# wielgosz-info/pedestrians-video-2-carla

Measured on AMD Instinct MI355X. Metric: clips/sec (B=256,T=16,J=26) pose_lifting train step, higher is better.
Workload: dtype f32; 1 GPU; flow=pose_lifting movements_model=LinearAE(pose_changes) loss=loc_2d_3d transform=hips_neck_bbox clip_length=16 J=26 batch_size=256/GPU (BASELINE.json metric config; configs[1]/[3] = --batch-size 1024); global_batch=256, per_gpu_batch=256, parallelism=dp1, hip_graph=True, lean_train_outputs=True, deferred_loss_finalize=True, two_launch_step=True, direct_replay=True, grad_allreduce_bytes=70120

## Files before the change

pedestrians_video_2_carla_amd/csrc/p2c_pose_head_dev.h:

```cpp
#pragma once
#include <hip/hip_runtime.h>
#include <stdint.h>
#include <math.h>

#include "../../include/p2c.h"

namespace p2c {

constexpr int J = P2C_JOINTS;
constexpr int GROUP = 32;
constexpr int IDL = 26;

static __constant__ int c_parent[GROUP] = {IDL, 0, 1, 2, 3, 4, 5, 6, 3, 8, 9, 9, 3, 12, 13, 14, 1, 16, 17, 18, 19, 1, 21, 22, 23, 24,
                                    26, 27, 28, 29, 30, 31};
static __constant__ int c_subtree_end[GROUP] = {25, 25, 15, 15, 7, 7, 7, 7, 11, 11, 10, 11, 15, 15, 15, 15, 20, 20, 20, 20, 20,
                                         25, 25, 25, 25, 25, 26, 27, 28, 29, 30, 31};
constexpr unsigned kInteriorMask = 0x3dee6feu;
static __constant__ int c_anc_r2[GROUP] = {26, 26, 0, 1, 2, 3, 4, 5, 3, 3, 8, 9, 3, 3, 12, 13, 1, 1, 16, 17, 18, 1, 1, 21, 22, 23,
                                    26, 27, 28, 29, 30, 31};
static __constant__ int c_anc_r3[GROUP] = {26, 26, 26, 26, 0, 1, 2, 3, 1, 1, 3, 3, 1, 1, 3, 3, 26, 26, 1, 1, 16, 26, 26, 1, 1, 21,
                                    26, 27, 28, 29, 30, 31};

struct V3 {
  float x, y, z;
// ... 61 lines not shown
#pragma unroll
  for (int i = 0; i < 9; ++i) c.m[i] = shfl(a.m[i], s);
  return c;
}
template <int CTRL, int ROW_MASK = 0xF>
__device__ __forceinline__ float dpp0(float v) {
  return __int_as_float(__builtin_amdgcn_update_dpp(0, __float_as_int(v), CTRL, ROW_MASK, 0xF, true));
}
__device__ __forceinline__ float group_prefix(float v) {
  v += dpp0<0x111>(v);
  v += dpp0<0x112>(v);
  v += dpp0<0x114>(v);
  v += dpp0<0x118>(v);
  v += dpp0<0x142, 0xA>(v);
  return v;
}
__device__ __forceinline__ float group_bcast(float v, int j, bool upper) {
  float lo = __int_as_float(__builtin_amdgcn_readlane(__float_as_int(v), j));
  float hi = __int_as_float(__builtin_amdgcn_readlane(__float_as_int(v), j + 32));
  return upper ? hi : lo;
}
__device__ __forceinline__ float group_sum(float v, bool upper) { return group_bcast(group_prefix(v), 31, upper); }
__device__ __forceinline__ float group_min(float v) {
#pragma unroll
  for (int d = 16; d >= 1; d >>= 1) v = fminf(v, __shfl_xor(v, d, 64));
  return v;
}
__device__ __forceinline__ float group_max(float v) {
#pragma unroll
  for (int d = 16; d >= 1; d >>= 1) v = fmaxf(v, __shfl_xor(v, d, 64));
  return v;
}
__device__ __forceinline__ float wave_sum(float v) {
#pragma unroll
  for (int d = 32; d >= 1; d >>= 1) v += __shfl_xor(v, d, 64);
  return v;
}

__device__ __forceinline__ float frcp(float x) { return __builtin_amdgcn_rcpf(x); }
__device__ __forceinline__ float fsqrt(float x) { return __builtin_amdgcn_sqrtf(x); }

__device__ __forceinline__ float nan_to_zero(float v) { return (isfinite(v)) ? v : 0.f; }

struct SixD {
  V3 a1, a2, b1, b2;
  float n1, n2, d;
  bool c1, c2;
};
__device__ __forceinline__ M3 rot6d_fwd(const float *y6, SixD &s) {
  s.a1 = v3(y6[0], y6[1], y6[2]);
  s.a2 = v3(y6[3], y6[4], y6[5]);
  float n1 = fsqrt(dot(s.a1, s.a1));
  s.c1 = n1 > 1e-12f;
  s.n1 = fmaxf(n1, 1e-12f);
  s.b1 = s.a1 * frcp(s.n1);
  s.d = dot(s.b1, s.a2);
  V3 u2 = s.a2 - s.b1 * s.d;
  float n2 = fsqrt(dot(u2, u2));
  s.c2 = n2 > 1e-12f;
  s.n2 = fmaxf(n2, 1e-12f);
  s.b2 = u2 * frcp(s.n2);
  V3 b3 = cross(s.b1, s.b2);
  return M3{{s.b1.x, s.b1.y, s.b1.z, s.b2.x, s.b2.y, s.b2.z, b3.x, b3.y, b3.z}};
}
__device__ __forceinline__ void rot6d_bwd(const SixD &s, const M3 &g, float *gy6) {
  V3 g1 = v3(g.m[0], g.m[1], g.m[2]), g2 = v3(g.m[3], g.m[4], g.m[5]), g3 = v3(g.m[6], g.m[7], g.m[8]);
  V3 gb1 = g1 + cross(s.b2, g3);
  V3 gb2 = g2 + cross(g3, s.b1);
// ... 64 lines not shown
    V3 l1 = vmul(l, Ra) + la;
    M3 R1 = mul(R, Ra);
    if (L.interior) {
      l = l1;
      R = R1;
    }
  }
  {
    M3 Ra = shfl(R, L.base + L.anc1);
    V3 la = shfl(l, L.base + L.anc1);
    l = vmul(l, Ra) + la;
    R = mul(R, Ra);
  }
  {
    M3 Ra = shfl(R, L.base + L.anc2);
    V3 la = shfl(l, L.base + L.anc2);
    l = vmul(l, Ra) + la;
    if (NEED_ROT) R = mul(R, Ra);
  }
}

struct World {
  M3 rot;
  V3 loc;
  bool on;
};

struct HeadAcc {
  float sum2, cnt2, sum3;
};

enum { MODE_FWD = 0, MODE_FWD_MATERIALIZE = 1, MODE_BWD = 2, MODE_TRAIN = 3 };

template <int MODE>
__device__ __forceinline__ V3 frame_head(const p2c_pose_head_desc &d, const LaneCtx &L, int t, V3 x, const World &W,
                                         HeadAcc &acc, float coef2, float coef3, const float *g_abs_ext,
                                         const float *g_projt_ext, const float *gt2v, const float *gt3v) {
  constexpr bool BWD = (MODE == MODE_BWD || MODE == MODE_TRAIN);
  constexpr bool SUMS = !BWD || MODE == MODE_TRAIN;
  constexpr bool MAT = (MODE == MODE_FWD_MATERIALIZE);
  const bool in_slice = (t >= d.t0) && (t < d.t1);
  const size_t frame = (size_t)L.clip * d.T + t;

  V3 w = v3(x.y, -x.x, x.z);
  V3 p = W.on ? vmul(w, W.rot) + W.loc : w;
  float Z = d.cam_dist - p.x;
  float invZ = frcp(Z);
  float u = d.cam_cx - d.cam_f * p.y * invZ;
  float v = d.cam_cy + d.cam_f * (p.z + d.cam_elev) * invZ;
  if (!L.active) { u = 0.f; v = 0.f; invZ = 0.f; }

  if (MAT) {
    if (L.active && d.out_projection_2d) {
      float *o = d.out_projection_2d + (frame * J + L.j) * 3;
      o[0] = u, o[1] = v, o[2] = invZ;
    }
    if (L.active && d.out_absolute_pose_loc) {
      float *o = d.out_absolute_pose_loc + (frame * J + L.j) * 3;
      o[0] = x.x, o[1] = x.y, o[2] = x.z;
    }
  }

  const int tr = d.transform;
  float su = 0.f, sv = 0.f, scale = 1.f;
  float hu = 0.f, hv = 0.f, ku = 0.f, kv = 0.f;
  float hn_scale = 1.f, bb_scale = 1.f;
  bool use_bb_scale = false;
  float minu = 0.f, maxu = 0.f, minv = 0.f, maxv = 0.f;
  bool missing = false;
  if (tr != P2C_TRANSFORM_NONE) {
    if (tr != P2C_TRANSFORM_BBOX) {
      const bool up = L.base != 0;
      hu = group_bcast(u, d.hips_idx[0], up);
      hv = group_bcast(v, d.hips_idx[0], up);
      if (d.n_hips == 2) {
        hu = 0.5f * (hu + group_bcast(u, d.hips_idx[1], up));
        hv = 0.5f * (hv + group_bcast(v, d.hips_idx[1], up));
      }
      ku = group_bcast(u, d.neck_idx[0], up);
      kv = group_bcast(v, d.neck_idx[0], up);
      if (d.n_neck == 2) {
        ku = 0.5f * (ku + group_bcast(u, d.neck_idx[1], up));
        kv = 0.5f * (kv + group_bcast(v, d.neck_idx[1], up));
      }
      float du = ku - hu, dv = kv - hv;
// ... 9 lines not shown
    }
    if (__any(need_bb)) {
      missing = !L.active || ((u < d.near_zero) && (v < d.near_zero)) || (L.j >= J);
      const float inf = __builtin_inff();
      minu = group_min(missing ? inf : u);
      minv = group_min(missing ? inf : v);
      maxu = group_max(missing ? -inf : u);
      maxv = group_max(missing ? -inf : v);
      float cu = 0.5f * (minu + maxu), cv = 0.5f * (minv + maxv);
      float top_v = fminf(minv, maxv);
      float dx = cu - cu, dy = top_v - cv;
      bb_scale = fsqrt(fmaf(dx, dx, dy * dy));
      if (tr == P2C_TRANSFORM_BBOX) {
        su = cu, sv = cv, scale = bb_scale;
      } else if (use_bb_scale) {
        scale = bb_scale * 0.5748f;
      }
    }
  }
  float nu = u, nv = v, wch = invZ;
  bool fin_u = true, fin_v = true, keep = true;
  float inv_scale = 1.f;
  if (tr != P2C_TRANSFORM_NONE) {
    inv_scale = frcp(scale);
    nu = (u - su) * inv_scale;
    nv = (v - sv) * inv_scale;
    fin_u = isfinite(nu), fin_v = isfinite(nv);
    nu = fin_u ? nu : 0.f;
    nv = fin_v ? nv : 0.f;
    wch = nan_to_zero(invZ);
    keep = wch >= d.near_zero;
    if (!keep) { nu = 0.f; nv = 0.f; }
  }
  if (MAT && tr != P2C_TRANSFORM_NONE && in_slice && L.clip < d.B) {
    if (L.active && d.out_projection_2d_transformed) {
      float *o = d.out_projection_2d_transformed + (frame * J + L.j) * 3;
      o[0] = nu, o[1] = nv, o[2] = wch;
    }
    if (L.j == 0) {
      if (d.out_shift) d.out_shift[frame * 2 + 0] = su, d.out_shift[frame * 2 + 1] = sv;
      if (d.out_scale) d.out_scale[frame] = scale;
    }
  }

  V3 gx = v3(0.f, 0.f, 0.f);
  float dnu = 0.f, dnv = 0.f;
  if (in_slice) {
    if (L.has2) {
      float g0 = gt2v[0], g1 = gt2v[1];
      bool m = !d.mask_missing_joints || L.never_masked || ((g0 != 0.f) && (g1 != 0.f));
      if (m) {
        float e0 = nu - g0, e1 = nv - g1;
        if (SUMS) {
          acc.sum2 += fmaf(e0, e0, e1 * e1);
          acc.cnt2 += 1.f;
        }
        if (BWD) {
          dnu = coef2 * e0;
          dnv = coef2 * e1;
        }
      }
    }
    if (L.has3) {
      float e0 = x.x - gt3v[0], e1 = x.y - gt3v[1], e2 = x.z - gt3v[2];
      if (SUMS) acc.sum3 += fmaf(e0, e0, fmaf(e1, e1, e2 * e2));
      if (BWD) gx = v3(coef3 * e0, coef3 * e1, coef3 * e2);
    }
  }
  if (!BWD) return gx;

  if (L.active && g_abs_ext) {
    const float *g = g_abs_ext + (frame * J + L.j) * 3;
    gx = gx + v3(g[0], g[1], g[2]);
  }
// ... 33 lines not shown
    if (tr == P2C_TRANSFORM_BBOX || __any(use_bb_scale)) {
      float g_minu = 0.f, g_maxu = 0.f, g_minv = 0.f, g_maxv = 0.f;
      if (tr == P2C_TRANSFORM_BBOX) {
        g_minu += 0.5f * gsu, g_maxu += 0.5f * gsu, g_minv += 0.5f * gsv, g_maxv += 0.5f * gsv;
      }
      if (tr == P2C_TRANSFORM_BBOX || use_bb_scale) {
        float dy = fminf(minv, maxv) - 0.5f * (minv + maxv);
        float g_dy = (bb_scale > 0.f) ? g_bbs * dy * frcp(bb_scale) : 0.f;
        g_minv += 0.5f * g_dy;
        g_maxv -= 0.5f * g_dy;
      }
      unsigned long long grp = 0xffffffffull << L.base;
      unsigned long long b;
      b = __ballot(!missing && u == minu) & grp;
      if (b && L.lane == __ffsll((long long)b) - 1) gu += g_minu;
      b = __ballot(!missing && u == maxu) & grp;
      if (b && L.lane == __ffsll((long long)b) - 1) gu += g_maxu;
      b = __ballot(!missing && v == minv) & grp;
      if (b && L.lane == __ffsll((long long)b) - 1) gv += g_minv;
      b = __ballot(!missing && v == maxv) & grp;
      if (b && L.lane == __ffsll((long long)b) - 1) gv += g_maxv;
    }
  }
  float fz = d.cam_f * invZ;
  float gb = -fz * gu;
  float gc = fz * gv;
  float gZ = (d.cam_f * p.y * gu - d.cam_f * (p.z + d.cam_elev) * gv) * invZ * invZ;
  V3 gp = v3(-gZ, gb, gc);
  V3 gw = W.on ? vmulT(gp, W.rot) : gp;
  if (L.active) gx = gx + v3(-gw.y, gw.x, gw.z);
  return gx;
}

__device__ __forceinline__ void world_step(const p2c_pose_head_desc &d, const LaneCtx &L, int t, World &W) {
  if (!W.on || L.clip >= d.B) return;
  size_t frame = (size_t)L.clip * d.T + t;
  if (d.drot) {
    M3 dr;
#pragma unroll
    for (int i = 0; i < 9; ++i) dr.m[i] = d.drot[frame * 9 + i];
    W.rot = d.world_absolute ? dr : mul(W.rot, dr);
  }
  if (d.dloc) {
    V3 dl = v3(d.dloc[frame * 3 + 0], d.dloc[frame * 3 + 1], d.dloc[frame * 3 + 2]);
    W.loc = d.world_absolute ? dl : W.loc + dl;
  }
}
__device__ __forceinline__ void world_store(const p2c_pose_head_desc &d, const LaneCtx &L, int t, const World &W) {
  if (L.j != 0 || L.clip >= d.B) return;
  size_t frame = (size_t)L.clip * d.T + t;
  if (d.out_world_loc) {
    d.out_world_loc[frame * 3 + 0] = W.loc.x, d.out_world_loc[frame * 3 + 1] = W.loc.y, d.out_world_loc[frame * 3 + 2] = W.loc.z;
  }
  if (d.out_world_rot) {
#pragma unroll
    for (int i = 0; i < 9; ++i) d.out_world_rot[frame * 9 + i] = W.rot.m[i];
  }
}

struct GradLosses {
  const float *p[3];
};
__device__ __forceinline__ void loss_coefs_n(const p2c_pose_head_desc &d, const GradLosses &gl, float n2, float n3,
                                             float &coef2, float &coef3) {
  if (!gl.p[0] && !gl.p[1] && !gl.p[2]) return;
  const float u0 = gl.p[0] ? *gl.p[0] : 0.f, u1 = gl.p[1] ? *gl.p[1] : 0.f, u2 = gl.p[2] ? *gl.p[2] : 0.f;
  float g2 = u0 + u2, g3 = u1 + u2;
// ... 112 lines not shown
typedef float fb_f32x4 __attribute__((ext_vector_type(4)));
template <int NY, int DIR>
__device__ __forceinline__ void load_frame(const LaneCtx &L, FramePtrs &p, FrameIn<NY> &f) {
  (void)L;
  if constexpr (NY == 6) {
    const fb_f32x4 a = __builtin_bit_cast(fb_f32x4, __builtin_amdgcn_raw_buffer_load_b128(p.y, p.oy, 0, 0));
    const fb_f32x2 b = __builtin_bit_cast(fb_f32x2, __builtin_amdgcn_raw_buffer_load_b64(p.y, p.oy + 16, 0, 0));
    f.y[0] = a[0], f.y[1] = a[1], f.y[2] = a[2], f.y[3] = a[3], f.y[4] = b[0], f.y[5] = b[1];
  } else if constexpr (NY == 9) {
    const fb_f32x4 a = __builtin_bit_cast(fb_f32x4, __builtin_amdgcn_raw_buffer_load_b128(p.y, p.oy, 0, 0));
    const fb_f32x4 b = __builtin_bit_cast(fb_f32x4, __builtin_amdgcn_raw_buffer_load_b128(p.y, p.oy + 16, 0, 0));
    const float c = __builtin_bit_cast(float, __builtin_amdgcn_raw_buffer_load_b32(p.y, p.oy + 32, 0, 0));
    f.y[0] = a[0], f.y[1] = a[1], f.y[2] = a[2], f.y[3] = a[3];
    f.y[4] = b[0], f.y[5] = b[1], f.y[6] = b[2], f.y[7] = b[3], f.y[8] = c;
  } else {
    static_assert(NY == 3, "frame inputs are 6-D rotations, 3x3 matrices or 3-D locations");
    const fb_f32x3 a = __builtin_bit_cast(fb_f32x3, __builtin_amdgcn_raw_buffer_load_b96(p.y, p.oy, 0, 0));
    f.y[0] = a[0], f.y[1] = a[1], f.y[2] = a[2];
  }
  const fb_f32x2 g2 = __builtin_bit_cast(fb_f32x2, __builtin_amdgcn_raw_buffer_load_b64(p.g2, p.o2, 0, 0));
  const fb_f32x3 g3 = __builtin_bit_cast(fb_f32x3, __builtin_amdgcn_raw_buffer_load_b96(p.g3, p.o3, 0, 0));
  f.g2[0] = g2[0], f.g2[1] = g2[1];
  f.g3[0] = g3[0], f.g3[1] = g3[1], f.g3[2] = g3[2];
  p.oy += DIR * p.sy, p.o2 += DIR * p.s2, p.o3 += DIR * p.s3;
}

__device__ __forceinline__ void store_m3(float *base, size_t idx, const M3 &a) {
  float *p = base + idx * 9;
#pragma unroll
  for (int i = 0; i < 9; ++i) p[i] = a.m[i];
}


__device__ __forceinline__ World world_at(const p2c_pose_head_desc &d, const LaneCtx &L, int t) {
  World W;
  W.on = (d.dloc != nullptr) || (d.drot != nullptr);
  W.rot = identity();
  W.loc = v3(0.f, 0.f, 0.f);
  if (W.on) {
    const int tt = t < d.T ? t : d.T - 1;
    if (d.world_absolute) world_step(d, L, tt, W);
    else
      for (int i = 0; i <= tt; ++i) world_step(d, L, i, W);
  }
  return W;
}

__device__ __forceinline__ M3 scan_time(M3 P, int t, int j, int T, float *planes, int plane_floats) {
  int cur = 0;
  for (int off = 1; off < T; off <<= 1) {
    float *mine = planes + cur * plane_floats + (t * GROUP + j) * 9;
#pragma unroll
    for (int i = 0; i < 9; ++i) mine[i] = P.m[i];
    __syncthreads();
    if (t >= off) {
      const float *q = planes + cur * plane_floats + ((t - off) * GROUP + j) * 9;
      M3 Q;
#pragma unroll
      for (int i = 0; i < 9; ++i) Q.m[i] = q[i];
      P = mul(P, Q);
    }
    cur ^= 1;
  }
  return P;
}

__device__ __forceinline__ float n3_elems(const p2c_pose_head_desc &d) {
// ... 42 lines not shown
```

pedestrians_video_2_carla_amd/csrc/p2c_train.hip:

```cpp
#include <hip/hip_runtime.h>
#include <stdlib.h>
#include <stdint.h>

#include "../../include/p2c.h"
#include "p2c_adam_math.h"
#include "p2c_mlp_dev.h"
#include "p2c_pose_head_dev.h"
#include "p2c_train_dev.h"

int p2c_internal_validate_pose_head(const p2c_pose_head_desc *d);

namespace p2c_train {

constexpr int T_MAX = TS;
constexpr int PLANE = T_MAX * ph::GROUP * 9;
constexpr int H_ROWS = S::h_off(NLAY);
constexpr int G_ROWS = S::act_rows() - S::h_off(1);
constexpr int ACT_FLOATS = (H_ROWS + G_ROWS) * TP;
static_assert((S::h_off(NLAY) - S::h_off(1)) * TP >= PLANE, "scan plane 1 aliases the rows of G_1 .. G_{L-1}");
static_assert(S::dim_at(NLAY) == ph::J * 6, "the last layer is the (26, 6) rotation output");
constexpr int SCRATCH = 64;
constexpr int LDS_FLOATS = S::w_total() + ACT_FLOATS + PLANE + SCRATCH;
static_assert(LDS_FLOATS * 4 <= 160 * 1024, "LDS budget");

// ... 38 lines not shown
}
__device__ __forceinline__ int image_ld(int l) {
  int r = 0;
#pragma unroll
  for (int i = 0; i < NLAY; ++i)
    if (i == l) r = S::ld(i);
  return r;
}

struct StaticTile {
  int l, ntile, mtile;
  int n_in, n_out;
  int g_row, h_row;
};
__host__ __device__ constexpr int tiles_m(int l) { return (S::dim_at(l) + 1 + 15) >> 4; }
__host__ __device__ constexpr int tiles_of(int l) { return ((S::dim_at(l + 1) + 15) >> 4) * tiles_m(l); }
__host__ __device__ constexpr int tile_start(int l) {
  int r = 0;
  for (int i = 0; i < l; ++i) r += tiles_of(i);
  return r;
}
__device__ __forceinline__ StaticTile locate_tile_static(int t) {
  StaticTile r{0, 0, 0, 0, 0, 0, 0};
#pragma unroll
  for (int i = 0; i < NLAY; ++i) {
    const bool in = (i == 0 || t >= tile_start(i)) && (i == NLAY - 1 || t < tile_start(i + 1));
    const int rem = t - tile_start(i), nt = rem / tiles_m(i);
    r.l = in ? i : r.l, r.ntile = in ? nt : r.ntile, r.mtile = in ? rem - nt * tiles_m(i) : r.mtile;
    r.n_in = in ? S::dim_at(i) : r.n_in, r.n_out = in ? S::dim_at(i + 1) : r.n_out;
    r.g_row = in ? f_g_off(i + 1) : r.g_row, r.h_row = in ? f_h_off(i) : r.h_row;
  }
  return r;
}
__device__ __forceinline__ ph::M3 scan_time2(ph::M3 P, int t, int j, int T, float *p0, float *p1) {
  float *cur = p0, *oth = p1;
  for (int off = 1; off < T; off <<= 1) {
    float *mine = cur + (t * ph::GROUP + j) * 9;
#pragma unroll
    for (int i = 0; i < 9; ++i) mine[i] = P.m[i];
    lds_barrier();
    if (t >= off) {
      const float *q = cur + ((t - off) * ph::GROUP + j) * 9;
      ph::M3 Q;
#pragma unroll
      for (int i = 0; i < 9; ++i) Q.m[i] = q[i];
      P = ph::mul(P, Q);
    }
    float *tmp = cur;
    cur = oth, oth = tmp;
  }
  return P;
}


#ifndef P2C_TRAIN_DMA_IMAGE
#define P2C_TRAIN_DMA_IMAGE 0
#endif
typedef __attribute__((address_space(3))) void *lds_void_ptr;
constexpr int IMG_CHUNKS = ((S::w_total() >> 2) + 63) / 64;
__device__ __forceinline__ void image_dma_issue(const float *w_image, float *lds, int wave, int lane) {
  const __amdgpu_buffer_rsrc_t rs = __builtin_amdgcn_make_buffer_rsrc(const_cast<float *>(w_image), 0, S::w_total() * 4, 0x00020000);
  const unsigned base = (unsigned)(uintptr_t)(lds_void_ptr)lds;
  constexpr int total4 = S::w_total() >> 2;
#pragma unroll
  for (int i = 0; i < (IMG_CHUNKS + WAVES - 1) / WAVES; ++i) {
    const int c = wave + i * WAVES;
// ... 44 lines not shown
    asm volatile("" : "+v"(clip));
    return d.skel_type[clip];
  };
  const int st_first = skel_type_of((int)blockIdx.x < d.B ? (int)blockIdx.x : 0);
  TileRegs xr;
  tile_issue<NTH>(m.x, (int64_t)blockIdx.x * T, (int64_t)blockIdx.x * T + T, S::dims(0), true, xr);
#if P2C_TRAIN_DMA_IMAGE
  image_dma_issue(m.w_image, lds, L.wave, L.lane);
#else
  ImageRegs wr;
  stage_issue(m.w_image, total4, wr, 0, 0, issue_mark<S>(1));
#endif
  ph::LaneCtx PL;
  PL.lane = threadIdx.x & 63, PL.j = PL.lane & 31, PL.base = PL.lane & 32, PL.clip = blockIdx.x;
  const int t = (int)(threadIdx.x >> 6) * 2 + (PL.lane >> 5);
  PL.active = (PL.j < ph::J) && (t < T);
  if (m.identity_maps) {
    PL.anc0 = ph::c_parent[PL.j], PL.anc1 = ph::c_anc_r2[PL.j], PL.anc2 = ph::c_anc_r3[PL.j];
    PL.interior = (ph::kInteriorMask >> PL.j) & 1u;
    PL.sub_end = ph::c_subtree_end[PL.j];
    PL.gm2 = PL.gm3 = (PL.j < ph::J) ? PL.j : -1;
    PL.never_masked = (PL.j == d.hips_lane);
    PL.has2 = PL.active && d.gt2d;
    PL.has3 = PL.active && d.gt3d;
  } else {
    ph::fill_lane(PL, d);
  }
  const int jc = PL.j < ph::J ? PL.j : 0, tc = t < T ? t : T - 1;
  typedef __attribute__((address_space(1))) const float gcfloat;
  uintptr_t ref_loc_lane = (uintptr_t)(d.ref_rel_loc + jc * 3), ref_rot_lane = (uintptr_t)(d.ref_rel_rot + jc * 9);
  asm volatile("" : "+v"(ref_loc_lane), "+v"(ref_rot_lane));
  const float c0raw = m.counts[(int)threadIdx.x < d.B ? threadIdx.x : 0];
  const float c1raw = m.counts[(int)threadIdx.x + NTH < d.B ? threadIdx.x + NTH : 0];
  if (blockIdx.x == 0 && (int)threadIdx.x < m.n_counters) m.counters[threadIdx.x] = 0;
  init_rows<NTH>(H, S::h_off(0) + S::dims(0), S::h_off(0) + k_rows(S::dims(0)), S::h_off(0) + S::dims(0));
  float coef2 = 0.f, coef3 = 0.f;
  float *red = scratch + 16;

  auto one_clip = [&](const int clip, int st, auto first_c) {
  constexpr bool first = decltype(first_c)::value;
  PL.clip = clip;
  if constexpr (!first) lds_barrier();
  float lraw[3], rraw[9];
  float g2raw[2], g3raw[3];
  {
    const size_t frame = (size_t)clip * T + tc;
    const float *b2 = d.gt2d ? d.gt2d : d.ref_rel_loc, *b3 = d.gt3d ? d.gt3d : d.ref_rel_loc;
    const float *p2 = b2 + (PL.has2 ? (frame * d.gt2d_joints + PL.gm2) * d.gt2d_channels : 0);
    const float *p3 = b3 + (PL.has3 ? (frame * d.gt3d_joints + PL.gm3) * 3 : 0);
    g2raw[0] = p2[0], g2raw[1] = p2[1];
    g3raw[0] = p3[0], g3raw[1] = p3[1], g3raw[2] = p3[2];
  }
  TT(0, 1);
  tile_commit<NTH>(S::dims(0), true, xr, H + S::h_off(0) * TP);
  {
    const int64_t nxt = (int64_t)clip + gridDim.x;
    tile_issue<NTH>(m.x, nxt * T, nxt < d.B ? nxt * T + T : 0, S::dims(0), true, xr);
  }
  static_assert(S::dims(2) + 1 <= 16 && S::dims(3) + 1 <= 16, "layers 1 and 2: one output tile each");
  static_assert(rounds_upto<S>(2) <= issue_mark<S>(2), "layer 2's image rounds are in flight before layer 1's barrier commits them");
  for_layers(sh, 0, nl, [&](int ll) {
    const bool run = ll == 2;
#if P2C_TRAIN_DMA_IMAGE
    if constexpr (first) image_dma_wait(ll == 1 ? 2 : ll, L.wave);
    if (run) lds_wave_sync();
    else lds_barrier();
    TT(0, 2 + ll);
#else
    if constexpr (first) {
      const int upto = ll == 1 ? 2 : ll;
      if (!run) stage_commit(total4, wr, lds, 0, ll == 0 ? 0 : rounds_upto<S>(ll - 1), rounds_upto<S>(upto));
    }
    if (run) lds_wave_sync();
    else lds_barrier();
    TT(0, 2 + ll);
    if constexpr (first) stage_issue(m.w_image, total4, wr, 0, issue_mark<S>(ll + 1), issue_mark<S>(ll + 2));
#endif
    if (ll == 0) {
      asm volatile("" : "+v"(st));
      gcfloat *pl = (gcfloat *)ref_loc_lane + (size_t)st * (ph::J * 3);
      lraw[0] = pl[0], lraw[1] = pl[1], lraw[2] = pl[2];
      gcfloat *pr = (gcfloat *)ref_rot_lane + (size_t)st * (ph::J * 9);
#pragma unroll
      for (int i = 0; i < 9; ++i) rraw[i] = K::SCAN ? pr[i] : 0.f;
    }
    const bool last = (ll == nl - 1);
    layer_forward<P2C_PREC_F32, true>(L, lds + S::w_off(ll), S::ld(ll), S::dims(ll), S::dims(ll + 1), !last, H + S::h_off(ll) * TP,
                  last ? Y : H + S::h_off(ll + 1) * TP, nullptr, false, false);
  });
  lds_barrier();
  TT(0, 8);

  float y6[6] = {1.f, 0.f, 0.f, 0.f, 1.f, 0.f};
  if (PL.active) {
#pragma unroll
    for (int i = 0; i < 6; ++i) y6[i] = Y[(PL.j * 6 + i) * TP + t];
  }
  const ph::V3 l = (PL.j < ph::J) ? ph::v3(lraw[0], lraw[1], lraw[2]) : ph::v3(0.f, 0.f, 0.f);
  ph::M3 Rref = ph::identity();
  if (K::SCAN && PL.j < ph::J) {
#pragma unroll
    for (int i = 0; i < 9; ++i) Rref.m[i] = rraw[i];
  }
  const float g2[2] = {PL.has2 ? g2raw[0] : 0.f, PL.has2 ? g2raw[1] : 0.f};
  const float g3[3] = {PL.has3 ? g3raw[0] : 0.f, PL.has3 ? g3raw[1] : 0.f, PL.has3 ? g3raw[2] : 0.f};
  if constexpr (first) {
    const float c0 = (int)threadIdx.x < d.B ? c0raw : 0.f, c1 = (int)threadIdx.x + NTH < d.B ? c1raw : 0.f;
    float cnt = c0 + c1;
    for (int i = threadIdx.x + 2 * NTH; i < d.B; i += NTH) cnt += m.counts[i];
#pragma unroll
    for (int o = 32; o >= 1; o >>= 1) cnt += __shfl_xor(cnt, o, 64);
    if (L.lane == 0) scratch[L.wave] = cnt;
  }
  ph::SixD s;
  const ph::M3 c = ph::rot6d_fwd(y6, s);
  ph::M3 R = c;
  if (K::SCAN) R = ph::mul(scan_time2(c, t, PL.j, T, plane0, plane1), Rref);
  else lds_barrier();
  TT(0, 9);
  if constexpr (first) {
    float n2 = 0.f;
    for (int w = 0; w < WAVES; ++w) n2 += scratch[w];
    ph::loss_coefs_n(d, gl, n2, ph::n3_elems(d), coef2, coef3);
  }
  ph::M3 A = R;
  ph::V3 x = l;
  ph::fk_doubling(PL, A, x);
  const ph::World W = ph::world_at(d, PL, t);
  ph::HeadAcc acc{0.f, 0.f, 0.f};
  ph::V3 F = ph::frame_head<ph::MODE_TRAIN>(d, PL, t, x, W, acc, coef2, coef3, nullptr, nullptr, g2, g3);
  TT(0, 10);
  {
    const float s2 = ph::wave_sum(acc.sum2), c2 = ph::wave_sum(acc.cnt2), s3 = ph::wave_sum(acc.sum3);
    if (L.lane == 0) red[L.wave * 3 + 0] = s2, red[L.wave * 3 + 1] = c2, red[L.wave * 3 + 2] = s3;
  }
  TT(0, 11);
  ph::V3 FX = ph::cross(F, x);
  ph::V3 PF = ph::v3(ph::group_prefix(F.x), ph::group_prefix(F.y), ph::group_prefix(F.z));
  ph::V3 PX = ph::v3(ph::group_prefix(FX.x), ph::group_prefix(FX.y), ph::group_prefix(FX.z));
  ph::V3 SubF = ph::shfl(PF, PL.base + PL.sub_end) - (PF - F);
  ph::V3 SubX = ph::shfl(PX, PL.base + PL.sub_end) - (PX - FX);
  ph::V3 tau = SubX - ph::cross(SubF, x);
  ph::V3 taup = ph::vmul(ph::vmulT(tau, A), R);
  ph::V3 g = taup;
  if (K::SCAN) {
    float *sb = plane0;
    lds_barrier();
    constexpr int ROW = ph::GROUP * 3, SUF_TILES = (ph::J * 3 + 15) / 16;
    static_assert(T_MAX == 16 && SUF_TILES <= WAVES && 16 * SUF_TILES <= ROW, "suffix sum over time: one 16-column tile per wave");
    const bool live = t < T;
    sb[(t * ph::GROUP + PL.j) * 3 + 0] = live ? taup.x : 0.f, sb[(t * ph::GROUP + PL.j) * 3 + 1] = live ? taup.y : 0.f;
    sb[(t * ph::GROUP + PL.j) * 3 + 2] = live ? taup.z : 0.f;
    lds_barrier();
    if (L.wave < SUF_TILES) {
      f32x4 su = {0.f, 0.f, 0.f, 0.f};
      float bv[4], av[4];
      int sc = L.c, sg = L.g;
      asm volatile("" : "+v"(sc), "+v"(sg));
#pragma unroll
      for (int u = 0; u < 4; ++u) {
        const int tt = 15 - 4 * u - sg;
        bv[u] = sb[tt * ROW + 16 * L.wave + sc], av[u] = tt >= sc ? 1.f : 0.f;
      }
// ... 15 lines not shown
      if (s.c1 && s.c2) {
        ph::V3 b3 = ph::v3(c.m[6], c.m[7], c.m[8]);
        float al = ph::dot(g, s.b1), be = ph::dot(g, s.b2), ga = ph::dot(g, b3);
        float r1 = ph::frcp(s.n1), r2 = ph::frcp(s.n2);
        float k3 = (be + al * s.d * r2) * r1, k2 = -ga * r1, k5 = -al * r2;
        gy6[0] = fmaf(k3, b3.x, k2 * s.b2.x), gy6[1] = fmaf(k3, b3.y, k2 * s.b2.y), gy6[2] = fmaf(k3, b3.z, k2 * s.b2.z);
        gy6[3] = k5 * b3.x, gy6[4] = k5 * b3.y, gy6[5] = k5 * b3.z;
      } else {
        ph::M3 Gm;
#pragma unroll
        for (int i = 0; i < 3; ++i) {
          ph::V3 ci = ph::v3(c.m[i * 3], c.m[i * 3 + 1], c.m[i * 3 + 2]);
          ph::V3 h = ph::cross(ci, g) * 0.5f;
          Gm.m[i * 3] = h.x, Gm.m[i * 3 + 1] = h.y, Gm.m[i * 3 + 2] = h.z;
        }
        ph::rot6d_bwd(s, Gm, gy6);
      }
    }
#pragma unroll
    for (int i = 0; i < 6; ++i) Y[(PL.j * 6 + i) * TP + t] = gy6[i];
  } else if (PL.j == ph::J) {
    for (int r = S::dims(nl); r < pad16(S::dims(nl)); ++r) Y[r * TP + t] = 0.f;
  }

  TT(0, 13);
  static_assert(S::dims(3) <= 16 && S::dims(2) <= 16, "dgrad steps 3 and 2: one m-tile each");
  for_layers_down(sh, nl - 1, 1, [&](int ll) {
    if (ll == 2) lds_wave_sync();
    else lds_barrier();
    TT(0, 14 + ll);
    layer_dgrad<P2C_PREC_F32, true>(L, lds + S::w_off(ll), S::ld(ll), S::dims(ll), S::dims(ll + 1), G + S::h_off(ll + 1) * TP, H + S::h_off(ll) * TP,
                G + S::h_off(ll) * TP);
  });
  lds_barrier();
  TT(0, 20);

  f32x4 *fdst = reinterpret_cast<f32x4 *>(m.factors) + (size_t)clip * F_ROWS * 4;
  auto put = [&](const float *src, f32x4 *dst, int rows) {
    for (int i = threadIdx.x; i < rows * 4; i += NTH) {
      const int o = (i >> 2) * TP + (i & 3) * 4;
      dst[i] = (f32x4){src[o], src[o + 1], src[o + 2], src[o + 3]};
    }
  };
  for_layers(sh, 0, nl, [&](int ll) { put(H + S::h_off(ll) * TP, fdst + f_h_off(ll) * 4, S::dims(ll)); });
  for_layers(sh, 0, nl, [&](int ll) { put(G + S::h_off(ll + 1) * TP, fdst + f_g_off(ll + 1) * 4, S::dims(ll + 1)); });
  if (threadIdx.x == 0) {
    float a = 0.f, b = 0.f, cc = 0.f;
    for (int w = 0; w < WAVES; ++w) a += red[w * 3], b += red[w * 3 + 1], cc += red[w * 3 + 2];
    float *pp = d.partials + (size_t)clip * 4;
    pp[0] = a, pp[1] = b, pp[2] = cc, pp[3] = 0.f;
  }
  TT(0, 39);
  };

  if ((int)blockIdx.x < d.B) one_clip((int)blockIdx.x, st_first, std::true_type{});
  for (int clip = (int)blockIdx.x + (int)gridDim.x; clip < d.B; clip += (int)gridDim.x)
    one_clip(clip, skel_type_of(clip), std::false_type{});
}

constexpr int WG_WAVES = 8, KS = 8;
struct WgradArgs {
  const float *factors;
  int32_t n_stiles, n_tiles_w;
  float *gW[NLAY], *gb[NLAY];
  float *w_image;
  float *slices;
  int32_t *counters;
  const float *loss_partials;
  float n3_elems;
  int32_t has2d, has3d;
  float *loss_sums, *losses;
};

__device__ __forceinline__ void finalize_losses(const WgradArgs &a, double (*sh)[256]) {
  double s0 = 0.0, s1 = 0.0, s2 = 0.0;
  const f32x4 *lp = reinterpret_cast<const f32x4 *>(a.loss_partials);
  for (int i0 = threadIdx.x; i0 < a.n_stiles; i0 += 8 * 256) {
    f32x4 v[8];
#pragma unroll
    for (int u = 0; u < 8; ++u) {
      const int i = i0 + u * 256;
      v[u] = lp[i < a.n_stiles ? i : 0];
    }
// ... 504 lines not shown
  if (adam) {
    o = *m.fused_adamw;
    if (!o.param || !o.grad || !o.exp_avg || !o.exp_avg_sq || !o.step || !o.ticket || !o.hyper) return P2C_E_NULL;
    int64_t n_params = 0;
    for (int l = 0; l < NLAY; ++l) {
      const float *lo = o.grad, *hi = o.grad + o.n;
      if (m.gW[l] < lo || m.gW[l] + (size_t)m.dims[l + 1] * m.dims[l] > hi || m.gb[l] < lo || m.gb[l] + m.dims[l + 1] > hi)
        return P2C_E_INDEX;
      n_params += (int64_t)m.dims[l + 1] * (m.dims[l] + 1);
    }
    if (n_params != o.n) return P2C_E_SHAPE;
  }
  hipStream_t stream = (hipStream_t)stream_;
  static bool attr_done = false;
  if (!attr_done) {
    (void)hipFuncSetAttribute((const void *)train_clip_kernel<P2C_KIND_POSE_CHANGES_6D>, hipFuncAttributeMaxDynamicSharedMemorySize, 160 * 1024);
    (void)hipFuncSetAttribute((const void *)train_clip_kernel<P2C_KIND_RELATIVE_ROT_6D>, hipFuncAttributeMaxDynamicSharedMemorySize, 160 * 1024);
    attr_done = true;
  }
  if (!m.skip_pack && (which & 1)) {
    rc = p2c_mlp_pack(&m, stream_);
    if (rc) return rc;
  }
  ph::GradLosses gl{{nullptr, nullptr, nullptr}};
  if (grad_losses_)
    for (int i = 0; i < 3; ++i) gl.p[i] = grad_losses_[i];
  int tiles = 0;
  for (int l = 0; l < NLAY; ++l) tiles += ((m.dims[l + 1] + 15) / 16) * ((m.dims[l] + 1 + 15) / 16);
  if (tiles != kTilesW) return P2C_E_SHAPE;
  float *slices = m.partials + (size_t)d.B * F_ROWS * 16;
  int32_t *counters = reinterpret_cast<int32_t *>(slices + (size_t)WS_BLOCKS_MAX * kTilesW * 256);
  int identity = 1;
  for (int j = 0; j < P2C_JOINTS; ++j) identity &= (d.gmap2d[j] == j) && (d.gmap3d[j] == j);
  ClipArgs ca{m.x, m.w_image, desc->pair_counts, m.partials, counters, tiles, identity};
  const size_t lds_a = (size_t)LDS_FLOATS * sizeof(float);
  hipError_t e = hipSuccess;
  const dim3 grid_a((unsigned)(d.B < kClipBlocks ? d.B : kClipBlocks));
  if ((which & 1) && d.B >= stream_min_b() && p2c_internal_train_stream_supported(d)) {
    rc = p2c_internal_train_stream_launch(d, gl, ca, stream);
    if (rc) return rc;
  } else if (which & 1) {
    if (d.kind == P2C_KIND_POSE_CHANGES_6D)
      hipLaunchKernelGGL(train_clip_kernel<P2C_KIND_POSE_CHANGES_6D>, grid_a, dim3(64 * WAVES), lds_a, stream, d, gl, ca);
    else
      hipLaunchKernelGGL(train_clip_kernel<P2C_KIND_RELATIVE_ROT_6D>, grid_a, dim3(64 * WAVES), lds_a, stream, d, gl, ca);
    e = hipGetLastError();
    if (e != hipSuccess) return (int)e;
  }
  if (!(which & 2)) return 0;

  WgradArgs wa{};
  wa.factors = m.partials, wa.n_stiles = d.B, wa.n_tiles_w = tiles;
  for (int l = 0; l < NLAY; ++l) wa.gW[l] = m.gW[l], wa.gb[l] = m.gb[l];
  wa.w_image = adam ? m.w_image : nullptr;
  wa.slices = slices, wa.counters = counters;
  wa.loss_partials = d.partials;
  wa.n3_elems = (float)((double)d.B * (double)(d.t1 - d.t0) * (double)d.n_common3d * 3.0);
  wa.has2d = d.gt2d ? 1 : 0, wa.has3d = d.gt3d ? 1 : 0;
  wa.loss_sums = d.loss_sums, wa.losses = d.losses;
  if (d.B >= wgrad_stream_min_b()) {
    int blocks = d.B / 8;
    static const int max_blocks = getenv("P2C_WGRAD_STREAM_BLOCKS") ? atoi(getenv("P2C_WGRAD_STREAM_BLOCKS")) : WS_BLOCKS_MAX;
    const int cap = max_blocks < WS_BLOCKS_MAX ? (max_blocks < 8 ? 8 : max_blocks) : WS_BLOCKS_MAX;
    blocks = blocks > cap ? cap : (blocks & ~7);
    if (blocks < 8) blocks = 8;
    static bool ws_attr = false;
    if (!ws_attr) {
      (void)hipFuncSetAttribute((const void *)wgrad_stream_kernel, hipFuncAttributeMaxDynamicSharedMemorySize, WS_SLOTS * WS_SLOT_FLOATS * 4);
      (void)hipGetLastError();
      ws_attr = true;
    }
    hipLaunchKernelGGL(wgrad_stream_kernel, dim3((unsigned)blocks), dim3(64 * WG_WAVES), WS_SLOTS * WS_SLOT_FLOATS * 4, stream, wa);
    e = hipGetLastError();
    if (e != hipSuccess) return (int)e;
    const dim3 grid_r((unsigned)(tiles * (64 / RED_L) + 1));
    if (adam) hipLaunchKernelGGL(wgrad_reduce_kernel<true>, grid_r, dim3(RED_L * RED_G), 0, stream, wa, blocks, o);
    else hipLaunchKernelGGL(wgrad_reduce_kernel<false>, grid_r, dim3(RED_L * RED_G), 0, stream, wa, blocks, o);
    e = hipGetLastError();
    return e == hipSuccess ? 0 : (int)e;
  }
  const dim3 grid_b((unsigned)(tiles * KS + 1));
  if (adam) hipLaunchKernelGGL(train_wgrad_kernel<true>, grid_b, dim3(64 * WG_WAVES), 0, stream, wa, o);
  else hipLaunchKernelGGL(train_wgrad_kernel<false>, grid_b, dim3(64 * WG_WAVES), 0, stream, wa, o);
  e = hipGetLastError();
  return e == hipSuccess ? 0 : (int)e;
}
```

pedestrians_video_2_carla_amd/csrc/p2c_train_dev.h:

```cpp
#pragma once
#include <hip/hip_runtime.h>
#include <stdint.h>

#include "../../include/p2c.h"
#include "p2c_mlp_dev.h"
#include "p2c_pose_head_dev.h"

namespace p2c_train {

using namespace p2c_mlp;
namespace ph = p2c;

using S = LinearAE156;
constexpr int NLAY = S::NLAY;
__host__ __device__ constexpr int f_h_off(int l) {
  int r = 0;
  for (int i = 0; i < l; ++i) r += S::dim_at(i);
  return r;
}
constexpr int F_HALF = f_h_off(NLAY);
__host__ __device__ constexpr int f_g_off(int l) {
  int r = F_HALF;
  for (int i = 1; i < l; ++i) r += S::dim_at(i);
  return r;
}
constexpr int F_ROWS = f_g_off(NLAY) + S::dim_at(NLAY);

struct ClipArgs {
  const float *x;
  const float *w_image;
  const float *counts;
  float *factors;
  int32_t *counters;
  int32_t n_counters;
  int32_t identity_maps;
};

}

bool p2c_internal_train_stream_supported(const p2c_pose_head_desc &d);
int p2c_internal_train_stream_launch(const p2c_pose_head_desc &d, const p2c::GradLosses &gl, const p2c_train::ClipArgs &m, hipStream_t stream);
```

Measured before the change: 9.877 million clips/s.

## Hoist loss-coefficient reduction into MLP forward and streamline per-clip factor store

Moves the pair-count reduction and loss-coefficient computation out of the post-forward critical path into idle slots during the forward layer loop, using a wave_sum rebuilt from permlane swaps and DPP. Pose-head constants are packed into a scalar-register struct so the head reads SGPRs instead of reloading the descriptor. The factor write-out becomes fully unrolled register-staged loads followed by stores, and the loss-partial write is done by wave 0. Prefetching gradient scales and precomputing n3_elems on the host adds register pressure and more complex indexing.

```diff
diff --git a/pedestrians_video_2_carla_amd/csrc/p2c_pose_head_dev.h b/pedestrians_video_2_carla_amd/csrc/p2c_pose_head_dev.h
--- a/pedestrians_video_2_carla_amd/csrc/p2c_pose_head_dev.h
+++ b/pedestrians_video_2_carla_amd/csrc/p2c_pose_head_dev.h
@@ -117,8 +117,22 @@
   return v;
 }
 __device__ __forceinline__ float wave_sum(float v) {
-#pragma unroll
-  for (int d = 32; d >= 1; d >>= 1) v += __shfl_xor(v, d, 64);
+  {
+    const auto r = __builtin_amdgcn_permlane32_swap(__float_as_uint(v), __float_as_uint(v), false, false);
+    v = __uint_as_float(r[0]) + __uint_as_float(r[1]);
+  }
+  {
+    const auto r = __builtin_amdgcn_permlane16_swap(__float_as_uint(v), __float_as_uint(v), false, false);
+    v = __uint_as_float(r[0]) + __uint_as_float(r[1]);
+  }
+  v += __int_as_float(__builtin_amdgcn_update_dpp(0, __float_as_int(v), 0x128, 0xF, 0xF, false));
+  {
+    int p = __builtin_amdgcn_update_dpp(0, __float_as_int(v), 0x104, 0xF, 0x5, false);
+    p = __builtin_amdgcn_update_dpp(p, __float_as_int(v), 0x114, 0xF, 0xA, false);
+    v += __int_as_float(p);
+  }
+  v += __int_as_float(__builtin_amdgcn_update_dpp(0, __float_as_int(v), 0x4E, 0xF, 0xF, false));
+  v += __int_as_float(__builtin_amdgcn_update_dpp(0, __float_as_int(v), 0xB1, 0xF, 0xF, false));
   return v;
 }
 
@@ -249,8 +263,8 @@
 
 enum { MODE_FWD = 0, MODE_FWD_MATERIALIZE = 1, MODE_BWD = 2, MODE_TRAIN = 3 };
 
-template <int MODE>
-__device__ __forceinline__ V3 frame_head(const p2c_pose_head_desc &d, const LaneCtx &L, int t, V3 x, const World &W,
+template <int MODE, class D>
+__device__ __forceinline__ V3 frame_head(const D &d, const LaneCtx &L, int t, V3 x, const World &W,
                                          HeadAcc &acc, float coef2, float coef3, const float *g_abs_ext,
                                          const float *g_projt_ext, const float *gt2v, const float *gt3v) {
   constexpr bool BWD = (MODE == MODE_BWD || MODE == MODE_TRAIN);
@@ -267,7 +281,7 @@
   float v = d.cam_cy + d.cam_f * (p.z + d.cam_elev) * invZ;
   if (!L.active) { u = 0.f; v = 0.f; invZ = 0.f; }
 
-  if (MAT) {
+  if constexpr (MAT) {
     if (L.active && d.out_projection_2d) {
       float *o = d.out_projection_2d + (frame * J + L.j) * 3;
       o[0] = u, o[1] = v, o[2] = invZ;
@@ -343,14 +357,16 @@
     keep = wch >= d.near_zero;
     if (!keep) { nu = 0.f; nv = 0.f; }
   }
-  if (MAT && tr != P2C_TRANSFORM_NONE && in_slice && L.clip < d.B) {
-    if (L.active && d.out_projection_2d_transformed) {
-      float *o = d.out_projection_2d_transformed + (frame * J + L.j) * 3;
-      o[0] = nu, o[1] = nv, o[2] = wch;
-    }
-    if (L.j == 0) {
-      if (d.out_shift) d.out_shift[frame * 2 + 0] = su, d.out_shift[frame * 2 + 1] = sv;
-      if (d.out_scale) d.out_scale[frame] = scale;
+  if constexpr (MAT) {
+    if (tr != P2C_TRANSFORM_NONE && in_slice && L.clip < d.B) {
+      if (L.active && d.out_projection_2d_transformed) {
+        float *o = d.out_projection_2d_transformed + (frame * J + L.j) * 3;
+        o[0] = nu, o[1] = nv, o[2] = wch;
+      }
+      if (L.j == 0) {
+        if (d.out_shift) d.out_shift[frame * 2 + 0] = su, d.out_shift[frame * 2 + 1] = sv;
+        if (d.out_scale) d.out_scale[frame] = scale;
+      }
     }
   }
 
@@ -450,7 +466,8 @@
   return gx;
 }
 
-__device__ __forceinline__ void world_step(const p2c_pose_head_desc &d, const LaneCtx &L, int t, World &W) {
+template <class D>
+__device__ __forceinline__ void world_step(const D &d, const LaneCtx &L, int t, World &W) {
   if (!W.on || L.clip >= d.B) return;
   size_t frame = (size_t)L.clip * d.T + t;
   if (d.drot) {
@@ -629,7 +646,8 @@
 }
 
 
-__device__ __forceinline__ World world_at(const p2c_pose_head_desc &d, const LaneCtx &L, int t) {
+template <class D>
+__device__ __forceinline__ World world_at(const D &d, const LaneCtx &L, int t) {
   World W;
   W.on = (d.dloc != nullptr) || (d.drot != nullptr);
   W.rot = identity();
diff --git a/pedestrians_video_2_carla_amd/csrc/p2c_train.hip b/pedestrians_video_2_carla_amd/csrc/p2c_train.hip
--- a/pedestrians_video_2_carla_amd/csrc/p2c_train.hip
+++ b/pedestrians_video_2_carla_amd/csrc/p2c_train.hip
@@ -94,6 +94,12 @@
   }
   return r;
 }
+struct PoseConsts {
+  typedef __attribute__((address_space(1))) const float gcfloat;
+  int32_t B, T, t0, t1, transform, n_hips, n_neck, hips_idx[2], neck_idx[2], mask_missing_joints, world_absolute;
+  float near_zero, cam_f, cam_cx, cam_cy, cam_dist, cam_elev;
+  gcfloat *dloc, *drot;
+};
 __device__ __forceinline__ ph::M3 scan_time2(ph::M3 P, int t, int j, int T, float *p0, float *p1) {
   float *cur = p0, *oth = p1;
   for (int off = 1; off < T; off <<= 1) {
@@ -204,10 +210,40 @@
   asm volatile("" : "+v"(ref_loc_lane), "+v"(ref_rot_lane));
   const float c0raw = m.counts[(int)threadIdx.x < d.B ? threadIdx.x : 0];
   const float c1raw = m.counts[(int)threadIdx.x + NTH < d.B ? threadIdx.x + NTH : 0];
+  float uraw[3];
+  {
+    uintptr_t up[3];
+#pragma unroll
+    for (int i = 0; i < 3; ++i) up[i] = (uintptr_t)(gl.p[i] ? gl.p[i] : m.counts);
+    asm volatile("" : "+v"(up[0]), "+v"(up[1]), "+v"(up[2]));
+#pragma unroll
+    for (int i = 0; i < 3; ++i) uraw[i] = *(gcfloat *)up[i];
+  }
   if (blockIdx.x == 0 && (int)threadIdx.x < m.n_counters) m.counters[threadIdx.x] = 0;
   init_rows<NTH>(H, S::h_off(0) + S::dims(0), S::h_off(0) + k_rows(S::dims(0)), S::h_off(0) + S::dims(0));
   float coef2 = 0.f, coef3 = 0.f;
   float *red = scratch + 16;
+  static_assert(WAVES >= 2 && 16 + 3 * WAVES <= SCRATCH && 2 * NTH <= PLANE, "scratch: coefficients, loss sums; plane 0: pair counts");
+
+  auto clip_pair_count = [&]() { plane0[threadIdx.x] = c0raw, plane0[threadIdx.x + NTH] = c1raw; };
+  auto clip_loss_coefs = [&]() {
+    float n2 = 0.f;
+#pragma unroll
+    for (int k = 0; k < 2 * NTH / 64; ++k) {
+      const float c = plane0[L.lane + 64 * k];
+      n2 += L.lane + 64 * k < d.B ? c : 0.f;
+    }
+    for (int i = L.lane + 2 * NTH; i < d.B; i += 64) n2 += m.counts[i];
+    n2 = ph::wave_sum(n2);
+    float k2 = 0.f, k3 = 0.f;
+    if (gl.p[0] || gl.p[1] || gl.p[2]) {
+      const float u0 = gl.p[0] ? uraw[0] : 0.f, u1 = gl.p[1] ? uraw[1] : 0.f, u2 = gl.p[2] ? uraw[2] : 0.f;
+      const float g2 = u0 + u2, g3 = u1 + u2, n3 = m.n3_elems;
+      k2 = (d.gt2d && n2 > 0.f) ? g2 / n2 : 0.f;
+      k3 = (d.gt3d && n3 > 0.f) ? 2.f * g3 / n3 : 0.f;
+    }
+    if (L.lane == 0) scratch[0] = k2, scratch[1] = k3;
+  };
 
   auto one_clip = [&](const int clip, int st, auto first_c) {
   constexpr bool first = decltype(first_c)::value;
@@ -231,10 +267,14 @@
   }
   static_assert(S::dims(2) + 1 <= 16 && S::dims(3) + 1 <= 16, "layers 1 and 2: one output tile each");
   static_assert(rounds_upto<S>(2) <= issue_mark<S>(2), "layer 2's image rounds are in flight before layer 1's barrier commits them");
+  PoseConsts pc;
   for_layers(sh, 0, nl, [&](int ll) {
     const bool run = ll == 2;
 #if P2C_TRAIN_DMA_IMAGE
     if constexpr (first) image_dma_wait(ll == 1 ? 2 : ll, L.wave);
+    if constexpr (first) {
+      if (ll == 1) clip_pair_count();
+    }
     if (run) lds_wave_sync();
     else lds_barrier();
     TT(0, 2 + ll);
@@ -243,11 +283,17 @@
       const int upto = ll == 1 ? 2 : ll;
       if (!run) stage_commit(total4, wr, lds, 0, ll == 0 ? 0 : rounds_upto<S>(ll - 1), rounds_upto<S>(upto));
     }
+    if constexpr (first) {
+      if (ll == 1) clip_pair_count();
+    }
     if (run) lds_wave_sync();
     else lds_barrier();
     TT(0, 2 + ll);
     if constexpr (first) stage_issue(m.w_image, total4, wr, 0, issue_mark<S>(ll + 1), issue_mark<S>(ll + 2));
 #endif
+    if constexpr (first) {
+      if (ll == 2 && L.wave == 1) clip_loss_coefs();
+    }
     if (ll == 0) {
       asm volatile("" : "+v"(st));
       gcfloat *pl = (gcfloat *)ref_loc_lane + (size_t)st * (ph::J * 3);
@@ -257,6 +303,15 @@
       for (int i = 0; i < 9; ++i) rraw[i] = K::SCAN ? pr[i] : 0.f;
     }
     const bool last = (ll == nl - 1);
+    if (last) {
+      pc = PoseConsts{d.B, d.T, d.t0, d.t1, d.transform, d.n_hips, d.n_neck, {d.hips_idx[0], d.hips_idx[1]}, {d.neck_idx[0], d.neck_idx[1]},
+                    d.mask_missing_joints, d.world_absolute, d.near_zero, d.cam_f, d.cam_cx, d.cam_cy, d.cam_dist, d.cam_elev,
+                    (PoseConsts::gcfloat *)d.dloc, (PoseConsts::gcfloat *)d.drot};
+      asm volatile("" : "+s"(pc.B), "+s"(pc.T), "+s"(pc.t0), "+s"(pc.t1), "+s"(pc.transform), "+s"(pc.n_hips), "+s"(pc.n_neck),
+                   "+s"(pc.hips_idx[0]), "+s"(pc.hips_idx[1]), "+s"(pc.neck_idx[0]), "+s"(pc.neck_idx[1]), "+s"(pc.mask_missing_joints));
+      asm volatile("" : "+s"(pc.world_absolute), "+s"(pc.near_zero), "+s"(pc.cam_f), "+s"(pc.cam_cx), "+s"(pc.cam_cy), "+s"(pc.cam_dist),
+                   "+s"(pc.cam_elev), "+s"(pc.dloc), "+s"(pc.drot));
+    }
     layer_forward<P2C_PREC_F32, true>(L, lds + S::w_off(ll), S::ld(ll), S::dims(ll), S::dims(ll + 1), !last, H + S::h_off(ll) * TP,
                   last ? Y : H + S::h_off(ll + 1) * TP, nullptr, false, false);
   });
@@ -276,31 +331,19 @@
   }
   const float g2[2] = {PL.has2 ? g2raw[0] : 0.f, PL.has2 ? g2raw[1] : 0.f};
   const float g3[3] = {PL.has3 ? g3raw[0] : 0.f, PL.has3 ? g3raw[1] : 0.f, PL.has3 ? g3raw[2] : 0.f};
-  if constexpr (first) {
-    const float c0 = (int)threadIdx.x < d.B ? c0raw : 0.f, c1 = (int)threadIdx.x + NTH < d.B ? c1raw : 0.f;
-    float cnt = c0 + c1;
-    for (int i = threadIdx.x + 2 * NTH; i < d.B; i += NTH) cnt += m.counts[i];
-#pragma unroll
-    for (int o = 32; o >= 1; o >>= 1) cnt += __shfl_xor(cnt, o, 64);
-    if (L.lane == 0) scratch[L.wave] = cnt;
-  }
+  if constexpr (first) coef2 = scratch[0], coef3 = scratch[1];
   ph::SixD s;
   const ph::M3 c = ph::rot6d_fwd(y6, s);
   ph::M3 R = c;
   if (K::SCAN) R = ph::mul(scan_time2(c, t, PL.j, T, plane0, plane1), Rref);
   else lds_barrier();
   TT(0, 9);
-  if constexpr (first) {
-    float n2 = 0.f;
-    for (int w = 0; w < WAVES; ++w) n2 += scratch[w];
-    ph::loss_coefs_n(d, gl, n2, ph::n3_elems(d), coef2, coef3);
-  }
   ph::M3 A = R;
   ph::V3 x = l;
   ph::fk_doubling(PL, A, x);
-  const ph::World W = ph::world_at(d, PL, t);
+  const ph::World W = ph::world_at(pc, PL, t);
   ph::HeadAcc acc{0.f, 0.f, 0.f};
-  ph::V3 F = ph::frame_head<ph::MODE_TRAIN>(d, PL, t, x, W, acc, coef2, coef3, nullptr, nullptr, g2, g3);
+  ph::V3 F = ph::frame_head<ph::MODE_TRAIN>(pc, PL, t, x, W, acc, coef2, coef3, nullptr, nullptr, g2, g3);
   TT(0, 10);
   {
     const float s2 = ph::wave_sum(acc.sum2), c2 = ph::wave_sum(acc.cnt2), s3 = ph::wave_sum(acc.sum3);
@@ -382,23 +425,40 @@
     layer_dgrad<P2C_PREC_F32, true>(L, lds + S::w_off(ll), S::ld(ll), S::dims(ll), S::dims(ll + 1), G + S::h_off(ll + 1) * TP, H + S::h_off(ll) * TP,
                 G + S::h_off(ll) * TP);
   });
+  uintptr_t part_p = (uintptr_t)(d.partials + (size_t)clip * 4);
+  asm volatile("" : "+s"(part_p));
   lds_barrier();
   TT(0, 20);
 
   f32x4 *fdst = reinterpret_cast<f32x4 *>(m.factors) + (size_t)clip * F_ROWS * 4;
-  auto put = [&](const float *src, f32x4 *dst, int rows) {
-    for (int i = threadIdx.x; i < rows * 4; i += NTH) {
-      const int o = (i >> 2) * TP + (i & 3) * 4;
-      dst[i] = (f32x4){src[o], src[o + 1], src[o + 2], src[o + 3]};
-    }
-  };
-  for_layers(sh, 0, nl, [&](int ll) { put(H + S::h_off(ll) * TP, fdst + f_h_off(ll) * 4, S::dims(ll)); });
-  for_layers(sh, 0, nl, [&](int ll) { put(G + S::h_off(ll + 1) * TP, fdst + f_g_off(ll + 1) * 4, S::dims(ll + 1)); });
-  if (threadIdx.x == 0) {
+  constexpr int F_ITEMS = F_ROWS * 4, F_ROUNDS = (F_ITEMS + NTH - 1) / NTH;
+  f32x4 fv[F_ROUNDS];
+#pragma unroll
+  for (int k = 0; k < F_ROUNDS; ++k) {
+    int i = threadIdx.x + k * NTH;
+    if ((k + 1) * NTH > F_ITEMS) i = i < F_ITEMS ? i : F_ITEMS - 1;
+    const int hi = ((k + 1) * NTH - 1) >> 2;
+    const int o = f_lds_row(i >> 2, (k * NTH) >> 2, hi < F_ROWS ? hi : F_ROWS - 1) * TP + (i & 3) * 4;
+    fv[k] = (f32x4){H[o], H[o + 1], H[o + 2], H[o + 3]};
+  }
+  float rv[3 * WAVES];
+  if (L.wave == 0) {
+#pragma unroll
+    for (int i = 0; i < 3 * WAVES; ++i) rv[i] = red[i];
+  }
+#pragma unroll
+  for (int k = 0; k < F_ROUNDS; ++k) {
+    const int i = threadIdx.x + k * NTH;
+    if ((k + 1) * NTH <= F_ITEMS || i < F_ITEMS) fdst[i] = fv[k];
+  }
+  if (L.wave == 0) {
     float a = 0.f, b = 0.f, cc = 0.f;
-    for (int w = 0; w < WAVES; ++w) a += red[w * 3], b += red[w * 3 + 1], cc += red[w * 3 + 2];
-    float *pp = d.partials + (size_t)clip * 4;
-    pp[0] = a, pp[1] = b, pp[2] = cc, pp[3] = 0.f;
+#pragma unroll
+    for (int w = 0; w < WAVES; ++w) a += rv[w * 3], b += rv[w * 3 + 1], cc += rv[w * 3 + 2];
+    if (L.lane == 0) {
+      __attribute__((address_space(1))) float *pp = (__attribute__((address_space(1))) float *)part_p;
+      pp[0] = a, pp[1] = b, pp[2] = cc, pp[3] = 0.f;
+    }
   }
   TT(0, 39);
   };
@@ -969,7 +1029,8 @@
   int32_t *counters = reinterpret_cast<int32_t *>(slices + (size_t)WS_BLOCKS_MAX * kTilesW * 256);
   int identity = 1;
   for (int j = 0; j < P2C_JOINTS; ++j) identity &= (d.gmap2d[j] == j) && (d.gmap3d[j] == j);
-  ClipArgs ca{m.x, m.w_image, desc->pair_counts, m.partials, counters, tiles, identity};
+  const float n3_elems = (float)((double)d.B * (double)(d.t1 - d.t0) * (double)d.n_common3d * 3.0);
+  ClipArgs ca{m.x, m.w_image, desc->pair_counts, m.partials, counters, tiles, identity, n3_elems};
   const size_t lds_a = (size_t)LDS_FLOATS * sizeof(float);
   hipError_t e = hipSuccess;
   const dim3 grid_a((unsigned)(d.B < kClipBlocks ? d.B : kClipBlocks));
@@ -992,7 +1053,7 @@
   wa.w_image = adam ? m.w_image : nullptr;
   wa.slices = slices, wa.counters = counters;
   wa.loss_partials = d.partials;
-  wa.n3_elems = (float)((double)d.B * (double)(d.t1 - d.t0) * (double)d.n_common3d * 3.0);
+  wa.n3_elems = n3_elems;
   wa.has2d = d.gt2d ? 1 : 0, wa.has3d = d.gt3d ? 1 : 0;
   wa.loss_sums = d.loss_sums, wa.losses = d.losses;
   if (d.B >= wgrad_stream_min_b()) {
diff --git a/pedestrians_video_2_carla_amd/csrc/p2c_train_dev.h b/pedestrians_video_2_carla_amd/csrc/p2c_train_dev.h
--- a/pedestrians_video_2_carla_amd/csrc/p2c_train_dev.h
+++ b/pedestrians_video_2_carla_amd/csrc/p2c_train_dev.h
@@ -34,7 +34,23 @@
   int32_t *counters;
   int32_t n_counters;
   int32_t identity_maps;
+  float n3_elems;
 };
+
+__host__ __device__ constexpr int f_seg_start(int s) { return s < NLAY ? f_h_off(s) : f_g_off(s - NLAY + 1); }
+__host__ __device__ constexpr int f_seg_lds_row(int s) {
+  return s < NLAY ? S::h_off(s) : S::h_off(NLAY) - S::h_off(1) + S::h_off(s - NLAY + 1);
+}
+__device__ __forceinline__ int f_lds_row(int r, int lo, int hi) {
+  int shift = 0;
+#pragma unroll
+  for (int s = 1; s < 2 * NLAY; ++s) {
+    const int d = f_seg_lds_row(s) - f_seg_start(s);
+    if (f_seg_start(s) <= lo) shift = d;
+    else if (f_seg_start(s) <= hi) shift = r >= f_seg_start(s) ? d : shift;
+  }
+  return r + shift;
+}
 
 }
 
```

Measured after the change: 10.11 million clips/s (median of 6 runs). +2.4%, better.
